# zchuning/repo

Measured on AMD Instinct MI355X. Metric: world-model+imagine updates/sec (B=50,L=50,64x64x3), higher is better.
Workload: dtype f32

## Files before the change

repo_amd/csrc/bconv.h:

```cpp
#pragma once
#include "bgemm.h"
#include "dconv.h"

namespace repo {

template <class G>
struct BGeo {
  static constexpr int KSE = G::KS + (G::KS & 1);
  static constexpr int TAPS = G::KS * KSE;
  static constexpr int KKE = (TAPS + 7) & ~7;
  static constexpr int BPG = KKE / 8;
  static constexpr bool ODD = (G::WB & 1) != 0;
  static constexpr int WBE = ODD ? ((G::WB + 3) & ~3) : G::WB;
  static constexpr int CBP = G::CB + (G::CB & 1);
};

template <int BM_, int BN_, int CK_, int WM_, int WN_>
struct BTile {
  static constexpr int BM = BM_, BN = BN_, CK = CK_, WM = WM_, WN = WN_;
  static constexpr int TM = BM / (32 * WM), TN = BN / (32 * WN);
  static constexpr int NT = WM * WN * 64;
  static_assert(TM >= 1 && TN >= 1 && BM % (32 * WM) == 0 && BN % (32 * WN) == 0 && CK % 2 == 0, "tile / wave grid mismatch");
};

template <class G, class T>
struct BPack {
  static constexpr int NBLK = (T::CK / 2) * BGeo<G>::BPG;
  static constexpr int NSL = BGeo<G>::CBP / T::CK;
  static constexpr int MT = (G::CS + T::BM - 1) / T::BM;
  static constexpr int WPLANE = NBLK * 2 * T::BM * 16;
  static constexpr int CHUNK_BYTES = 3 * WPLANE;
  static constexpr size_t BYTES = (size_t)MT * NSL * CHUNK_BYTES;
  static constexpr size_t BYTES_U8 = BYTES + (size_t)((G::CS * 4 + 255) & ~255);
  static_assert(BGeo<G>::CBP % T::CK == 0, "channel chunk must divide the (pair-padded) channel count");
};

struct BPackArgs {
  const float* w;
  char* wp;
  const float* bias;
};

template <class G, class T, bool U8 = false>
__global__ __launch_bounds__(256) void bconv_pack_kernel(BPackArgs p) {
  typedef BGeo<G> BG;
  typedef BPack<G, T> P;
  const int total = P::MT * P::NSL * P::NBLK * 2 * T::BM;
  if (U8) {
    float* fb = reinterpret_cast<float*>(p.wp + P::BYTES);
    for (int cs = blockIdx.x * 256 + threadIdx.x; cs < G::CS; cs += gridDim.x * 256) {
      double s = 0.0;
      for (int k = 0; k < G::CB * G::KK; ++k) s += (double)p.w[(size_t)cs * G::CB * G::KK + k];
      fb[cs] = (float)((double)(p.bias ? p.bias[cs] : 0.f) - s);
    }
  }
  for (int i = blockIdx.x * 256 + threadIdx.x; i < total; i += gridDim.x * 256) {
    int r = i;
    const int m = r % T::BM;
    r /= T::BM;
    const int h = r & 1;
    r >>= 1;
    const int blk = r % P::NBLK;
    r /= P::NBLK;
    const int t = r % P::NSL, mt = r / P::NSL;
    const int g = blk / BG::BPG, b = blk % BG::BPG;
    const int cs = mt * T::BM + m, cb = t * T::CK + 2 * g + h;
    float v[8];
#pragma unroll
    for (int j = 0; j < 8; ++j) {
      const int q = 8 * b + j, ky = q / BG::KSE, kx = q % BG::KSE;
      v[j] = (q < BG::TAPS && kx < G::KS && cs < G::CS && cb < G::CB) ? p.w[((size_t)cs * G::CB + cb) * G::KK + ky * G::KS + kx] : 0.f;
      if (U8) v[j] *= 2.f / 255.f;
    }
    unsigned pl[3][4];
#pragma unroll
    for (int e = 0; e < 4; ++e) bg_split3(v[2 * e], v[2 * e + 1], pl[0][e], pl[1][e], pl[2][e]);
    char* dst = p.wp + ((size_t)mt * P::NSL + t) * P::CHUNK_BYTES + ((blk * 2 + h) * T::BM + m) * 16;
#pragma unroll
    for (int q3 = 0; q3 < 3; ++q3)
      *reinterpret_cast<u32x4s*>(dst + q3 * P::WPLANE) = u32x4s{pl[q3][0], pl[q3][1], pl[q3][2], pl[q3][3]};
  }
}

template <class G, class T, class BigT = float, int NPROD = 6>
__global__ __launch_bounds__(T::NT) void bconv_down_kernel(DownArgs p) {
  typedef BGeo<G> BG;
  typedef BPack<G, T> P;
  constexpr bool U8 = std::is_same<BigT, uint8_t>::value;
  static_assert(U8 ? (NPROD == 3 || NPROD == 2) : (NPROD == 6 || NPROD == 3), "products per block");
  constexpr int NWPL = U8 ? NPROD : BgProd<U8 ? 6 : NPROD>::PLANES;
  constexpr int NPL = U8 ? 1 : NWPL;
  static_assert(BG::CBP == G::CB || P::NSL == 1, "a padded channel count: one chunk (the phantom channel is chunk-local)");
  static_assert(!U8 || !BG::ODD, "uint8 frames: even row pitch");
  constexpr bool ODD = BG::ODD;
  constexpr int WBE = BG::WBE;
  constexpr int BM = T::BM, BN = T::BN, CK = T::CK, NT = T::NT, TM = T::TM, TN = T::TN;
  constexpr int NBLK = P::NBLK, NSL = P::NSL, WPLANE = P::WPLANE;
  constexpr int ROWS_FULL = 2 * (G::HS - 1) + G::KS;
  constexpr int LENFULL = (ROWS_FULL * G::WB + 3) & ~3;
  constexpr int NIMG_MAX = (BN - 1) / G::PS + 2;
  constexpr int PLMAX = cmin(NIMG_MAX * LENFULL,
                             ((2 * (BN / G::WS + 2) + NIMG_MAX * (G::KS - 2)) * G::WB + 4 * NIMG_MAX + 3) & ~3);
  constexpr int PLV = PLMAX / 4;
  constexpr int LENFULL_E = ODD ? ROWS_FULL * WBE : LENFULL;
  constexpr int PLMAX_E = ODD ? cmin(NIMG_MAX * LENFULL_E, ((2 * (BN / G::WS + 2) + NIMG_MAX * (G::KS - 2)) * WBE + 3) & ~3)
                              : PLMAX;
  constexpr int PPLANE = (CK * PLMAX_E * 2 + 15) & ~15;
  constexpr bool QROW = ODD;
  static_assert(!ODD || WBE % 4 == 0, "padded pitch: whole quads per row");
  constexpr int PLV_E = PLMAX_E / 4;
  constexpr int W_NV = NWPL * NBLK * 2 * BM;
  constexpr int W_PER = (W_NV + NT - 1) / NT, P_PER = (CK * (QROW ? PLV_E : PLV) + NT - 1) / NT;
  constexpr int EPI_FLOATS = (NT / 64) * 32 * 36 + (NT / 64) * TM * 32;
  constexpr int LDS_BYTES = cmax(3 * WPLANE + (U8 ? 1 : 3) * PPLANE + 64, 4 * EPI_FLOATS);
  __shared__ __attribute__((aligned(16))) char lds[LDS_BYTES];
  char* Wl = lds;
  char* Pl = lds + 3 * WPLANE;

  const int tid = threadIdx.x;
  const int lane = tid & 63;
  const int wid = __builtin_amdgcn_readfirstlane(tid >> 6);
  const int wm = wid / T::WN, wn = wid % T::WN;
  const int li = lane & 31, lh = lane >> 5;

  const int Ntot = p.nimg * G::PS;
  const int n0 = xcd_tile(blockIdx.x, gridDim.x) * BN, m0 = blockIdx.y * BM;
  const int nlast = min(n0 + BN, Ntot) - 1;
  const int ia = n0 / G::PS, ib = nlast / G::PS;
  const int fa = (n0 % G::PS) / G::WS, lb = (nlast % G::PS) / G::WS;
  const int la_ = (ia == ib) ? lb : G::HS - 1;
  const int lenA = ((2 * (la_ - fa) + G::KS) * G::WB + 3) & ~3;
  auto span_start = [&](int i) __attribute__((always_inline)) { return i == ia ? 0 : lenA + (i - ia - 1) * LENFULL; };
  const int PL = span_start(ib) + (ib == ia ? lenA : ((2 * lb + G::KS) * G::WB + 3) & ~3);
  const int lenA_e = (2 * (la_ - fa) + G::KS) * WBE;
  auto span_start_e = [&](int i) __attribute__((always_inline)) {
    return ODD ? (i == ia ? 0 : lenA_e + (i - ia - 1) * LENFULL_E) : span_start(i);
  };

  const __amdgpu_buffer_rsrc_t rbig = make_rsrc(p.big, p.big_bytes), rw = make_rsrc(p.w, p.w_bytes);

  unsigned poff[P_PER];
  int plds[P_PER];
#pragma unroll
  for (int j = 0; j < P_PER; ++j) {
    if (QROW) {
      const int v = tid + j * NT, c = v / PLV_E, qe = (v % PLV_E) * 4;
      int i, rel;
      if (qe < lenA_e) {
        i = ia;
        rel = qe;
      } else {
        i = ia + 1 + (qe - lenA_e) / LENFULL_E;
        rel = (qe - lenA_e) % LENFULL_E;
      }
      const int rows_i = (i == ia) ? 2 * (la_ - fa) + G::KS : (i == ib ? 2 * lb + G::KS : ROWS_FULL);
      const int r = rel / WBE, col = rel % WBE;
      const bool act = c < CK && i <= ib && r < rows_i;
      const int f = (i == ia) ? fa : 0;
      poff[j] = act ? 4u * (unsigned)((i * G::CB + c) * G::PB + (2 * f + r) * G::WB + col) : kOobOffset;
      plds[j] = act ? 2 * (c * PLMAX_E + span_start_e(i) + rel) : -1;
      continue;
    }
    const int v = tid + j * NT, c = v / PLV, q = (v % PLV) * 4;
    const bool act = c < CK && q < PL;
    int i, rel;
    if (q < lenA) {
      i = ia;
      rel = q;
    } else {
      i = ia + 1 + (q - lenA) / LENFULL;
      rel = (q - lenA) % LENFULL;
    }
    const int f = (i == ia) ? fa : 0;
    poff[j] = (act && c < G::CB) ? (unsigned)sizeof(BigT) * (unsigned)((i * G::CB + c) * G::PB + 2 * f * G::WB + rel) : kOobOffset;
    plds[j] = act ? 2 * (c * PLMAX_E + q) : -1;
  }
  constexpr unsigned P_STEP = (unsigned)sizeof(BigT) * CK * G::PB;
  const unsigned wbase = (unsigned)(blockIdx.y * NSL) * (unsigned)P::CHUNK_BYTES;

  int bbh[TN];
#pragma unroll
  for (int j = 0; j < TN; ++j) {
    const int n = min(n0 + (wn * TN + j) * 32 + li, Ntot - 1);
    const int i = n / G::PS, pix = n % G::PS;
    const int f = (i == ia) ? fa : 0;
    bbh[j] = 2 * (span_start_e(i) + 2 * (pix / G::WS - f) * WBE + 2 * (pix % G::WS) + lh * PLMAX_E);
  }
  const int abase = (lh * BM + wm * (TM * 32) + li) * 16;

  f32x16 acc[TM][TN];
#pragma unroll
  for (int i = 0; i < TM; ++i)
#pragma unroll
    for (int j = 0; j < TN; ++j)
#pragma unroll
      for (int r = 0; r < 16; ++r) acc[i][j][r] = 0.f;

  f32x4 rwv[W_PER];
  typename Patch4<BigT>::raw_t rpv[P_PER];
  auto gload = [&](int t) __attribute__((always_inline)) {
#pragma unroll
    for (int j = 0; j < W_PER; ++j) {
      const int v = tid + j * NT;
      rwv[j] = VecLoad<4>::load(rw, ((W_NV % NT == 0) || v < W_NV) ? wbase + (unsigned)t * P::CHUNK_BYTES + 16u * v : kOobOffset);
    }
#pragma unroll
    for (int j = 0; j < P_PER; ++j)
      rpv[j] = Patch4<BigT>::load(rbig, poff[j] == kOobOffset ? kOobOffset : poff[j] + (unsigned)t * P_STEP);
  };
  auto lstore = [&]() __attribute__((always_inline)) {
#pragma unroll
    for (int j = 0; j < W_PER; ++j) {
      const int v = tid + j * NT;
      if ((W_NV % NT == 0) || v < W_NV) *reinterpret_cast<f32x4*>(Wl + 16 * v) = rwv[j];
    }
#pragma unroll
    for (int j = 0; j < P_PER; ++j)
      if (plds[j] >= 0) {
        if constexpr (U8) {
          const unsigned v = rpv[j];
          const unsigned f0 = __builtin_bit_cast(unsigned, (float)(v & 0xffu)), f1 = __builtin_bit_cast(unsigned, (float)((v >> 8) & 0xffu));
          const unsigned f2 = __builtin_bit_cast(unsigned, (float)((v >> 16) & 0xffu)), f3 = __builtin_bit_cast(unsigned, (float)(v >> 24));
          *reinterpret_cast<bg_u32x2*>(Pl + plds[j]) = bg_u32x2{(f0 >> 16) | (f1 & 0xffff0000u), (f2 >> 16) | (f3 & 0xffff0000u)};
        } else {
          unsigned a1, a2, a3, b1, b2, b3;
          bg_split3(rpv[j][0], rpv[j][1], a1, a2, a3);
          bg_split3(rpv[j][2], rpv[j][3], b1, b2, b3);
          *reinterpret_cast<bg_u32x2*>(Pl + plds[j]) = bg_u32x2{a1, b1};
          *reinterpret_cast<bg_u32x2*>(Pl + PPLANE + plds[j]) = bg_u32x2{a2, b2};
          if constexpr (NPL > 2) *reinterpret_cast<bg_u32x2*>(Pl + 2 * PPLANE + plds[j]) = bg_u32x2{a3, b3};
        }
      }
  };
  auto qoff = [](int g, int q) constexpr {
    const int ky = q / BG::KSE, kx = q % BG::KSE;
    return (q < BG::TAPS && kx < G::KS) ? 2 * (2 * g * PLMAX_E + ky * WBE + kx) : 2 * (2 * g * PLMAX_E);
  };
  auto compute = [&]() __attribute__((always_inline)) {
#pragma unroll
    for (int blk = 0; blk < NBLK; ++blk) {
      const int g = blk / BG::BPG, b = blk % BG::BPG;
      bg_bf16x8 fa[TM][3], fb[TN][NPL];
#pragma unroll
      for (int pl = 0; pl < NWPL; ++pl) {
#pragma unroll
        for (int i = 0; i < TM; ++i)
          fa[i][pl] = *reinterpret_cast<const bg_bf16x8*>(Wl + pl * WPLANE + blk * (2 * BM * 16) + abase + i * 32 * 16);
#pragma unroll
        for (int j = 0; j < (pl < NPL ? TN : 0); ++j) {
          const char* pb = Pl + pl * PPLANE + bbh[j];
          u32x4s d;
#pragma unroll
          for (int pp = 0; pp < 4; ++pp) d[pp] = *reinterpret_cast<const unsigned*>(pb + qoff(g, 8 * b + 2 * pp));
          fb[j][pl] = __builtin_bit_cast(bg_bf16x8, d);
        }
      }
#pragma unroll
      for (int i = 0; i < TM; ++i)
#pragma unroll
        for (int j = 0; j < TN; ++j) {
          f32x16 c = acc[i][j];
          if constexpr (U8) {
            if constexpr (NPROD == 3) c = __builtin_amdgcn_mfma_f32_32x32x16_bf16(fa[i][2], fb[j][0], c, 0, 0, 0);
            c = __builtin_amdgcn_mfma_f32_32x32x16_bf16(fa[i][1], fb[j][0], c, 0, 0, 0);
            c = __builtin_amdgcn_mfma_f32_32x32x16_bf16(fa[i][0], fb[j][0], c, 0, 0, 0);
          } else if constexpr (NPROD == 3) {
            c = __builtin_amdgcn_mfma_f32_32x32x16_bf16(fa[i][0], fb[j][1], c, 0, 0, 0);
            c = __builtin_amdgcn_mfma_f32_32x32x16_bf16(fa[i][1], fb[j][0], c, 0, 0, 0);
            c = __builtin_amdgcn_mfma_f32_32x32x16_bf16(fa[i][0], fb[j][0], c, 0, 0, 0);
          } else {
            c = __builtin_amdgcn_mfma_f32_32x32x16_bf16(fa[i][1], fb[j][NPL > 1 ? 1 : 0], c, 0, 0, 0);
            c = __builtin_amdgcn_mfma_f32_32x32x16_bf16(fa[i][0], fb[j][NPL > 2 ? 2 : 0], c, 0, 0, 0);
            c = __builtin_amdgcn_mfma_f32_32x32x16_bf16(fa[i][2], fb[j][0], c, 0, 0, 0);
            c = __builtin_amdgcn_mfma_f32_32x32x16_bf16(fa[i][0], fb[j][NPL > 1 ? 1 : 0], c, 0, 0, 0);
            c = __builtin_amdgcn_mfma_f32_32x32x16_bf16(fa[i][1], fb[j][0], c, 0, 0, 0);
            c = __builtin_amdgcn_mfma_f32_32x32x16_bf16(fa[i][0], fb[j][0], c, 0, 0, 0);
          }
          acc[i][j] = c;
        }
    }
  };

  gload(0);
  if (ODD) {
    for (int i = tid; i < NPL * PPLANE / 16; i += NT) reinterpret_cast<f32x4*>(Pl)[i] = f32x4{0.f, 0.f, 0.f, 0.f};
    __syncthreads();
  }
  lstore();
  __syncthreads();
  for (int t = 0; t < NSL; ++t) {
    if (t + 1 < NSL) gload(t + 1);
#ifndef BC_NO_COMPUTE
    compute();
#endif
    __syncthreads();
    if (t + 1 < NSL) {
#ifndef BC_NO_STAGE
      lstore();
#endif
      __syncthreads();
    }
  }
  dconv_down_epilogue<G, T>(p, reinterpret_cast<float*>(lds), acc, n0, m0, Ntot);
}

template <class G, class T, class BigT = float, int NPROD = 6>
inline int launch_bconv_down(const DownArgs& a, const float* w, char* pack, hipStream_t s) {
  typedef BPack<G, T> P;
  constexpr bool U8 = std::is_same<BigT, uint8_t>::value;
  const int total = P::MT * P::NSL * P::NBLK * 2 * T::BM;
  hipLaunchKernelGGL((bconv_pack_kernel<G, T, U8>), dim3((unsigned)((total + 255) / 256)), dim3(256), 0, s, BPackArgs{w, pack, a.bias});
  hipError_t e = hipGetLastError();
  if (e != hipSuccess) return (int)e;
  DownArgs b = a;
  b.w = reinterpret_cast<const float*>(pack);
  b.w_bytes = (unsigned)P::BYTES;
  if (U8) b.bias = reinterpret_cast<const float*>(pack + P::BYTES);
  const long gx = ((long)a.nimg * G::PS + T::BN - 1) / T::BN, gy = P::MT;
  hipLaunchKernelGGL((bconv_down_kernel<G, T, BigT, NPROD>), dim3((unsigned)gx, (unsigned)gy), dim3(T::NT), 0, s, b);
  e = hipGetLastError();
  return e == hipSuccess ? REPO_OK : (int)e;
}

}
```

repo_amd/csrc/conv.hip:

```cpp
#include <stdlib.h>
#include <string.h>

#include <algorithm>
#include <type_traits>

#include "igemm.h"
#include "dconv.h"
#include "uconv.h"
#include "dconv_up.h"
#include "bconv.h"
#include "buconv.h"
#include "bwgrad.h"
#include "bdec4.h"
#include "twgrad.h"
#include "tconv_up.h"
#include "tconv_down.h"

namespace repo {

static thread_local int t_bconv_enabled = 1;

static thread_local int t_conv_precision = -1;
static int env_conv_precision() {
  static const int mode = [] {
// ... 258 lines not shown
      float* p = dw + (size_t)m * Ncols + n;
      *p = accumulate ? *p + s : s;
    } else if (db) {
      db[m] = accumulate ? db[m] + s : s;
    }
  }
}

__global__ void partial_sum_rows_kernel(const float* __restrict__ parts, int n, float* __restrict__ out, float scale,
                                        int accumulate) {
  __shared__ float red[16];
  const float* row = parts + (size_t)blockIdx.x * n;
  float s = 0.f;
  for (int i = threadIdx.x; i < n; i += blockDim.x) s += row[i];
  s = block_sum(s, red);
  if (threadIdx.x == 0) out[blockIdx.x] = accumulate ? out[blockIdx.x] + scale * s : scale * s;
}

__global__ void partial_sum_kernel(const float* __restrict__ parts, int n, float* __restrict__ out, int accumulate) {
  __shared__ float red[16];
  float s = 0.f;
  for (int i = threadIdx.x; i < n; i += blockDim.x) s += parts[i];
  s = block_sum(s, red);
  if (threadIdx.x == 0) *out = accumulate ? *out + s : s;
}

__global__ void channel_sum_kernel(const float* __restrict__ x, int nimg, int C, int P, int imgs_per_split,
                                   float* __restrict__ parts) {
  __shared__ float red[16];
  const int c = blockIdx.x, s = blockIdx.y;
  const int i0 = s * imgs_per_split, i1 = min(nimg, i0 + imgs_per_split);
  const int nt = blockDim.x;
  const int dq = nt / P, dr = nt % P;
  int img = i0 + (int)threadIdx.x / P, p = (int)threadIdx.x % P;
  float a0 = 0.f, a1 = 0.f;
  const size_t cstride = (size_t)C * P;
  const float* base = x + (size_t)c * P;
  while (img < i1) {
    a0 += base[img * cstride + p];
    p += dr;
    img += dq;
    if (p >= P) {
      p -= P;
      ++img;
    }
    if (img >= i1) break;
    a1 += base[img * cstride + p];
    p += dr;
    img += dq;
    if (p >= P) {
      p -= P;
      ++img;
    }
  }
  const float acc = block_sum(a0 + a1, red);
  if (threadIdx.x == 0) parts[s * C + c] = acc;
}
__global__ void channel_sum_final_kernel(const float* __restrict__ parts, int splits, int C, float* __restrict__ out,
                                         int accumulate) {
  const int lane = threadIdx.x & 63;
  const int c = blockIdx.x * (blockDim.x >> 6) + (threadIdx.x >> 6);
  if (c >= C) return;
  float s = 0.f;
  for (int z = lane; z < splits; z += 64) s += parts[z * C + c];
  s = wave_sum(s);
  if (lane == 0) out[c] = accumulate ? out[c] + s : s;
}

__global__ void relu_mask_kernel(int64_t n, const float* __restrict__ dy, const float* __restrict__ h,
                                 float* __restrict__ y) {
  const int64_t stride = (int64_t)gridDim.x * blockDim.x;
  for (int64_t i = (int64_t)blockIdx.x * blockDim.x + threadIdx.x; i < n; i += stride) y[i] = h[i] > 0.f ? dy[i] : 0.f;
}

struct Off {};
template <class T> constexpr bool kOn = !std::is_same<T, Off>::value;

template <class Down_, class Wgrad_, int WGT_>
struct LayerFp32 {
  using Down = Down_; using Wgrad = Wgrad_; static constexpr int WGT = WGT_;
  using DownLat = Off;
  using DownBf = Off;
  using DownBfU8 = Off;
  using DownTcd = Off;
  static bool down_tcd_takes(int, bool, bool) { return false; }
  using UpScatter = Off;
  using UpBfScatter = Off;
  using DirectUp = Off;
  static constexpr bool UpTconv = false;
  using WgradBf = Off;
  static constexpr int TwNBK = 0, TwNPW = 4;
  static constexpr bool TwDbig = true;
};

template <class G> struct Layer;
template <> struct Layer<GEnc1> : LayerFp32<DTile<32, 512, 3, 1, 8>, WTile<32, 64, 1, 2, 1, 4, 2>, 3072> {
  using DownBfU8 = BTile<32, 512, 4, 1, 8>;
};
template <> struct Layer<GEnc2> : LayerFp32<DTile<64, 128, 2, 2, 2>, WTile<64, 128, 2, 2, 1, 7, 2>, 768> {
  using DownLat = DTile<32, 128, 4, 1, 4>;
  using DownBf = BTile<64, 256, 4, 1, 4>;
  using DownTcd = TcdGeoE2;
  static bool down_tcd_takes(int epi, bool, bool) { return epi == REPO_EPI_RELU; }
  using UpScatter = SConf<GEnc2, 1, 8>;
  using UpBfScatter = BSConf<GEnc2, 1, 4>;
  static constexpr bool UpTconv = true;
  static constexpr int TwNBK = 2, TwNPW = 8;
};
template <> struct Layer<GEnc3> : LayerFp32<DTile<128, 128, 2, 2, 2>, WTile<64, 128, 2, 2, 2, 6>, 1024> {
  using DownLat = DTile<32, 128, 8, 1, 4>;
  using DownBf = BTile<128, 128, 4, 2, 2>;
  using UpScatter = SConf<GEnc3, 4, 2>;
  using UpBfScatter = BSConf<GEnc3, 4, 4>;
  using WgradBf = WTile<64, 256, 1, 4, 1, 6>;
};
template <> struct Layer<GEnc4> : LayerFp32<DTile<32, 64, 2, 1, 2>, WTile<64, 128, 2, 2, 8, 2>, 768> {
  using DownLat = DTile<32, 128, 8, 1, 4>;
  using DownBf = BTile<128, 64, 4, 2, 2>;
  using UpScatter = SConf<GEnc4, 8, 1>;
  using UpBfScatter = BSConf<GEnc4, 8, 2>;
};
template <> struct Layer<GDec2> : LayerFp32<DTile<128, 128, 4, 2, 4, 1>, WTile<64, 128, 2, 2, 4, 5>, 1536> {
  using DownBf = BTile<64, 128, 2, 1, 4>;
  using UpScatter = SConf<GDec2, 5, 2>;
  using UpBfScatter = BSConf<GDec2, 5, 4>;
};
template <> struct Layer<GDec3> : LayerFp32<DTile<64, 128, 2, 2, 2>, WTile<64, 128, 2, 2, 1, 7>, 2048> {
  using DownBf = BTile<64, 256, 2, 1, 4>;
  using DownTcd = TcdGeo;
  static bool down_tcd_takes(int epi, bool has_bias, bool wants_cmask) {
    return (epi == REPO_EPI_NONE || epi == REPO_EPI_MUL_DRELU) && !has_bias && !wants_cmask;
  }
  using UpScatter = SConf<GDec3, 1, 6>;
  using UpBfScatter = BSConf<GDec3, 1, 4>;
  using WgradBf = WTile<64, 128, 1, 4, 1, 7>;
  static constexpr int TwNBK = 2;
};
template <> struct Layer<GDec4> : LayerFp32<DTile<32, 256, 3, 1, 8>, WTile<32, 128, 1, 4, 1, 2>, 1536> {};
template <> struct Layer<GX1> : LayerFp32<DTile<32, 512, 3, 1, 8>, WTile<32, 64, 1, 2, 1, 2, 2>, 3072> {};
template <> struct Layer<GX2> : LayerFp32<DTile<64, 128, 2, 2, 2>, WTile<64, 128, 2, 2, 1, 3, 2>, 1536> {
  using DirectUp = DTile<128, 128, 8, 2, 4>;
};
template <> struct Layer<GX3> : LayerFp32<DTile<128, 128, 2, 2, 2>, WTile<64, 128, 2, 2, 1, 7>, 1024> {
  using UpScatter = SConf<GX3, 1, 2>;
};
template <> struct Layer<GX4> : LayerFp32<DTile<64, 128, 2, 2, 2>, WTile<64, 128, 2, 2, 2, 6>, 1024> {
  using UpScatter = SConf<GX4, 4, 1>;
};
template <> struct Layer<GY4> : LayerFp32<DTile<32, 256, 2, 1, 4>, WTile<32, 128, 1, 4, 1, 2>, 1536> {
  using DirectUp = DTile<64, 256, 4, 2, 4>;
};
template <> struct Layer<GY5> : LayerFp32<DTile<32, 512, 3, 1, 8>, WTile<32, 64, 1, 2, 1, 2>, 1536> {};
template <> struct Layer<GT4> : LayerFp32<DTile<32, 256, 3, 1, 8>, WTile<32, 128, 1, 4, 1, 2>, 1536> {
  using DirectUp = DTile<32, 256, 4, 1, 8>;
};

template <class G> struct Route : Layer<G> {
#if defined(TCD_DISABLE)
  using DownTcd = Off;
#elif defined(TCD_NO_ENC2)
  using DownTcd = std::conditional_t<std::is_same<G, GEnc2>::value, Off, typename Layer<G>::DownTcd>;
#endif
#ifdef TCU_DISABLE
  static constexpr bool UpTconv = false;
#endif
#ifdef TW_DISABLE
  static constexpr int TwNBK = 0;
#endif
#ifdef TW_NO_DBIG
  static constexpr bool TwDbig = false;
#endif
};
template <class G> using DownLatTile = std::conditional_t<kOn<typename Route<G>::DownLat>, typename Route<G>::DownLat, typename Route<G>::Down>;
template <class G, class BigT> using DownBfTile = std::conditional_t<std::is_same<BigT, float>::value, typename Route<G>::DownBf, typename Route<G>::DownBfU8>;

constexpr size_t round256(size_t b) { return (b + 255) & ~(size_t)255; }

enum class DownEngine { Fp32Lat, Fp32, Bf16, Tcd };
struct DownPlan {
  DownEngine engine;
  long tiles;
  size_t pack_bytes;
  size_t parts_bytes;
  bool high;
  size_t need() const { return pack_bytes + parts_bytes; }
};
template <class G, class BigT>
static DownPlan down_plan(int64_t nimg, int epi, bool has_bias, bool wants_dbias, bool wants_cmask, size_t ws_have) {
  using R = Route<G>;
  using BT = DownBfTile<G, BigT>;
  const long px = nimg * (long)G::PS;
  auto plan = [&](DownEngine e, long bn, size_t pack) {
    const long tiles = (px + bn - 1) / bn;
    return DownPlan{e, tiles, pack, wants_dbias ? (size_t)tiles * G::CS * sizeof(float) : 0, conv_precision_high()};
  };
  if constexpr (kOn<BT>) {
    if (t_bconv_enabled && px > 512) {
      using P = BPack<G, BT>;
      constexpr size_t pack = round256(std::is_same<BigT, float>::value ? P::BYTES : P::BYTES_U8);
      DownPlan b = plan(DownEngine::Bf16, BT::BN, pack);
      if constexpr (kOn<typename R::DownTcd>) {
        static_assert(std::is_same<BigT, float>::value && R::DownTcd::PACK_BYTES <= pack,
                      "tconv_down: float frames; its pack fits the room of the bf16x6 kernel's");
        if (nimg >= 32 && !wants_dbias && R::down_tcd_takes(epi, has_bias, wants_cmask)) b.engine = DownEngine::Tcd;
      }
      if (ws_have >= b.need()) return b;
    }
  }
  return px <= 512 ? plan(DownEngine::Fp32Lat, DownLatTile<G>::BN, 0) : plan(DownEngine::Fp32, R::Down::BN, 0);
}
template <class G>
static size_t conv_down_ws_bytes(int64_t nimg) {
  const DownPlan f = down_plan<G, float>(nimg, REPO_EPI_NONE, false, true, false, SIZE_MAX);
  const DownPlan u = down_plan<G, uint8_t>(nimg, REPO_EPI_NONE, false, true, false, SIZE_MAX);
  return std::max(f.pack_bytes, u.pack_bytes) + std::max(f.parts_bytes, u.parts_bytes);
}

template <class G, class BigT>
static int conv_down_t(int64_t nimg, const BigT* big, const float* w, const float* bias, float* small, int epi,
                       const float* aux, float* dbias, int accumulate_dbias, unsigned char* cmask, void* ws,
                       size_t ws_bytes, hipStream_t s) {
  if (cmask && G::CS % 4 != 0) return REPO_E_BADARG;
  if (nimg * (int64_t)G::CB * G::PB >= kMaxBufElems || nimg * (int64_t)G::CS * G::PS >= kMaxBufElems) return REPO_E_SHAPE;
  const size_t ws_have = ws ? ws_bytes : 0;
  const DownPlan p = down_plan<G, BigT>(nimg, epi, bias != nullptr, dbias != nullptr, cmask != nullptr, ws_have);
  if (ws_have < p.need()) return REPO_E_WS_TOO_SMALL;
  float* parts = dbias ? (float*)((char*)ws + p.pack_bytes) : nullptr;
  DownArgs a{big, w, bias, aux, small, (int)nimg, epi, (unsigned)(nimg * G::CB * G::PB * sizeof(BigT)),
             (unsigned)(G::CS * G::CB * G::KK * sizeof(float)), parts, cmask};
  int rc = REPO_E_BADARG;
  switch (p.engine) {
    case DownEngine::Tcd:
      if constexpr (kOn<typename Route<G>::DownTcd>)
        rc = p.high ? launch_tconv_down<typename Route<G>::DownTcd, 3>(a, w, (char*)ws, s)
                    : launch_tconv_down<typename Route<G>::DownTcd, 6>(a, w, (char*)ws, s);
      break;
    case DownEngine::Bf16:
      if constexpr (kOn<DownBfTile<G, BigT>>) {
        constexpr int NFULL = std::is_same<BigT, float>::value ? 6 : 3;
        rc = p.high ? launch_bconv_down<G, DownBfTile<G, BigT>, BigT, NFULL == 6 ? 3 : 2>(a, w, (char*)ws, s)
                    : launch_bconv_down<G, DownBfTile<G, BigT>, BigT, NFULL>(a, w, (char*)ws, s);
      }
      break;
    case DownEngine::Fp32Lat: rc = launch_dconv_down<G, BigT, DownLatTile<G>>(a, s); break;
    case DownEngine::Fp32: rc = launch_dconv_down<G, BigT, typename Route<G>::Down>(a, s); break;
  }
  if (rc || !dbias) return rc;
  hipLaunchKernelGGL(channel_sum_final_kernel, dim3(cdiv(G::CS, 4)), dim3(256), 0, s, (const float*)parts, (int)p.tiles,
                     (int)G::CS, dbias, accumulate_dbias);
  REPO_CHECK_LAUNCH();
  return REPO_OK;
}

enum class UpEngine { Tconv, BfScatter, Direct, Scatter, Merged };
struct UpPlan {
  UpEngine engine;
  UpEngine base;
  bool tcu_live;
  size_t tcu_off;
  size_t need;
  size_t total;
  bool high;
};
template <class G>
static UpPlan up_plan(int64_t nimg, int epi, size_t ws_have) {
  using R = Route<G>;
  using UC = typename R::UpScatter;
  using BC = typename R::UpBfScatter;
  static_assert(!kOn<BC> || kOn<UC>, "the bf16x6 scatter kernel has an fp32 twin (repo_debug_bconv(0))");
  static_assert(!kOn<typename R::DirectUp> || !kOn<UC>, "the direct kernel or the scatter kernels");
  static_assert(!R::UpTconv || kOn<BC>, "the gather-form kernel follows the debug switch of the bf16x6 kernels");
  UpPlan p{UpEngine::Merged, UpEngine::Merged, false, 0, 0, 0, conv_precision_high()};
  size_t room = 0;
  if constexpr (kOn<BC>) {
    p.base = t_bconv_enabled ? UpEngine::BfScatter : UpEngine::Scatter;
    p.need = t_bconv_enabled ? BC::PACK_BYTES : UC::PACK_FLOATS * sizeof(float);
    room = std::max(BC::PACK_BYTES, UC::PACK_FLOATS * sizeof(float));
  } else if constexpr (kOn<typename R::DirectUp>) {
    p.base = UpEngine::Direct, p.need = room = UpGeo<G>::PACK_FLOATS * sizeof(float);
  } else if constexpr (kOn<UC>) {
    p.base = UpEngine::Scatter, p.need = room = UC::PACK_FLOATS * sizeof(float);
  }
  p.engine = p.base;
  p.tcu_off = round256(room);
  p.total = R::UpTconv ? p.tcu_off + kTcuPackBytes : room;
  p.tcu_live = R::UpTconv && t_bconv_enabled;
  const bool epi_ok = epi == REPO_EPI_NONE || epi == REPO_EPI_MUL_DRELU || epi == REPO_EPI_MUL_CMASK;
  if (p.tcu_live && epi_ok && nimg >= 4 && ws_have >= p.total) {
    p.engine = UpEngine::Tconv;
    p.need = p.total;
  }
  return p;
}

template <class G>
static int conv_up_pack_t(const float* w, void* ws, size_t ws_bytes, hipStream_t s) {
  using R = Route<G>;
  const size_t ws_have = ws ? ws_bytes : 0;
  const UpPlan p = up_plan<G>(0, REPO_EPI_NONE, ws_have);
  if (ws_have < (p.tcu_live ? p.total : p.need)) return REPO_E_WS_TOO_SMALL;
  if (p.tcu_live)
    if (const int rc = launch_tconv_up_pack(w, (char*)ws + p.tcu_off, s)) return rc;
  if constexpr (kOn<typename R::UpBfScatter>)
    if (p.base == UpEngine::BfScatter) return launch_buconv_pack<G, typename R::UpBfScatter>(w, ws, ws_bytes, s);
  if constexpr (kOn<typename R::DirectUp>) return launch_dconv_up_pack<G>(w, ws, ws_bytes, s);
  else if constexpr (kOn<typename R::UpScatter>) return launch_uconv_pack<G, typename R::UpScatter>(w, ws, ws_bytes, s);
  else return REPO_OK;
}

template <class G>
static int conv_up_t(int64_t nimg, const float* small, const float* w, const float* bias, float* big, int epi,
                     const float* aux, int packed, void* ws, size_t ws_bytes, hipStream_t s) {
  if (nimg * (int64_t)G::CB * G::PB >= kMaxBufElems || nimg * (int64_t)G::CS * G::PS >= kMaxBufElems) return REPO_E_SHAPE;
  using R = Route<G>;
  if (epi == REPO_EPI_MUL_CMASK && (!kOn<typename R::UpScatter> || G::CB % 4 != 0)) return REPO_E_BADARG;
  if (epi == REPO_EPI_FILM_RELU && !kOn<typename R::UpScatter>) return REPO_E_BADARG;
  const size_t ws_have = ws ? ws_bytes : 0;
  const UpPlan p = up_plan<G>(nimg, epi, ws_have);
  if (ws_have < p.need) return REPO_E_WS_TOO_SMALL;
  if constexpr (R::UpTconv)
    if (p.engine == UpEngine::Tconv) {
      char* pack = (char*)ws + p.tcu_off;
// ... 369 lines not shown
```

repo_amd/csrc/dconv.h:

```cpp
#pragma once
#include "vgemm.h"

namespace repo {

template <int BM_, int BN_, int CK_, int WM_, int WN_, int LDWPAD_ = 2>
struct DTile {
  static constexpr int BM = BM_, BN = BN_, CK = CK_, WM = WM_, WN = WN_, LDWPAD = LDWPAD_;
  static constexpr int TM = BM / (32 * WM), TN = BN / (32 * WN);
  static constexpr int NT = WM * WN * 64;
  static_assert(TM >= 1 && TN >= 1 && BM % (32 * WM) == 0 && BN % (32 * WN) == 0, "tile / wave grid mismatch");
};

#ifdef REPO_IGEMM_STAMPS
#define REPO_STAMP_FLUSH(nslices)                                              \
  do {                                                                         \
    REPO_STAMP(4);                                                             \
    if ((threadIdx.x & 63) == 0 && blockIdx.x % 16 == 0) {                     \
      for (int i_ = 0; i_ < 6; ++i_) atomicAdd(&g_igemm_stamps[i_], st_[i_]);  \
      atomicAdd(&g_igemm_stamps[6], 1ull);                                     \
      atomicAdd(&g_igemm_stamps[7], (unsigned long long)(nslices));            \
    }                                                                          \
  } while (0)
#else
#define REPO_STAMP_FLUSH(nslices)
// ... 100 lines not shown
            float fsc = 1.f, fsh = 0.f;
            if (p.epi == REPO_EPI_FILM_RELU) {
              fsc = p.aux[(size_t)(2 * img) * G::CS + m];
              fsh = p.aux[(size_t)(2 * img + 1) * G::CS + m];
            }
#pragma unroll
            for (int e = 0; e < 4; ++e) {
              float x = v[e] + bv;
              if (p.epi == REPO_EPI_RELU) x = fmaxf(x, 0.f);
              else if (p.epi == REPO_EPI_MUL_DRELU || p.epi == REPO_EPI_MUL_MASK4) x = a4[e] > 0.f ? x : 0.f;
              else if (p.epi == REPO_EPI_FILM_RELU) x = fmaxf(fmaf(fsc, x, fsh), 0.f);
              v[e] = x;
            }
            qs = (v[0] + v[1]) + (v[2] + v[3]);
            __builtin_amdgcn_raw_buffer_store_b128(__builtin_bit_cast(u32x4s, v), rout, 4u * o, 0, 0);
          } else {
#pragma unroll
            for (int e = 0; e < 4; ++e) {
              const int ne = n + e;
              if (ne < Ntot) {
                const int oe = ((ne / G::PS) * G::CS + m) * G::PS + ne % G::PS;
                float x = v[e] + bv;
                if (p.epi == REPO_EPI_RELU) x = fmaxf(x, 0.f);
                else if (p.epi == REPO_EPI_FILM_RELU)
                  x = fmaxf(fmaf(p.aux[(size_t)(2 * (ne / G::PS)) * G::CS + m], x, p.aux[(size_t)(2 * (ne / G::PS) + 1) * G::CS + m]), 0.f);
                else if (p.epi == REPO_EPI_MUL_DRELU) x = p.aux[oe] > 0.f ? x : 0.f;
                else if (p.epi == REPO_EPI_MUL_MASK4)
                  x = (reinterpret_cast<const unsigned char*>(p.aux)[oe >> 2] >> (oe & 3)) & 1 ? x : 0.f;
                p.out[oe] = x;
                qs += x;
              }
            }
          }
        }
        if (p.chan_part) {
          qs += __shfl_xor(qs, 1, 64);
          qs += __shfl_xor(qs, 2, 64);
          qs += __shfl_xor(qs, 4, 64);
          csum[i][pass] += qs;
        }
      }
      if (p.cmask) {
        const int cq = lane >> 3, q = lane & 7;
        const int m4 = mt + 4 * cq, n = nb + 4 * q;
        if (m4 < G::CS && n < Ntot) {
          f32x4 rws[4];
          float bq[4];
#pragma unroll
          for (int c = 0; c < 4; ++c) {
            rws[c] = *reinterpret_cast<const f32x4*>(strip + (4 * cq + c) * EP + 4 * q);
            bq[c] = p.bias ? p.bias[m4 + c] : 0.f;
          }
#pragma unroll
          for (int e = 0; e < 4; ++e) {
            const int ne = n + e;
            if (ne < Ntot) {
              unsigned bits = 0;
#pragma unroll
              for (int c = 0; c < 4; ++c) bits |= (rws[c][e] + bq[c] > 0.f ? 1u : 0u) << c;
              p.cmask[((size_t)(ne / G::PS) * (G::CS / 4) + (m4 >> 2)) * G::PS + ne % G::PS] = (unsigned char)bits;
            }
          }
        }
      }
      __builtin_amdgcn_wave_barrier();
    }
  if (p.chan_part) {
    float* red = lds + (NT / 64) * 32 * EP;
    if ((lane & 7) == 0) {
#pragma unroll
      for (int i = 0; i < TM; ++i)
#pragma unroll
        for (int pass = 0; pass < 4; ++pass) red[wid * (TM * 32) + i * 32 + pass * 8 + (lane >> 3)] = csum[i][pass];
    }
    __syncthreads();
    if (tid < BM && m0 + tid < G::CS) {
      const int wmc = tid / (TM * 32), c = tid % (TM * 32);
      float t = 0.f;
#pragma unroll
      for (int x = 0; x < T::WN; ++x) t += red[(wmc * T::WN + x) * (TM * 32) + c];
      p.chan_part[(size_t)blockIdx.x * G::CS + m0 + tid] = t;
    }
  }
}

template <class G, class BigT, class T>
__global__ __launch_bounds__(T::NT) void dconv_down_kernel(DownArgs p) {
  constexpr int BM = T::BM, BN = T::BN, CK = T::CK, NT = T::NT, TM = T::TM, TN = T::TN;
  constexpr int KSL = CK * G::KK;
  constexpr int NSL = G::CB / CK;
  static_assert(G::CB % CK == 0 && KSL % 4 == 0, "channel chunk must divide CB and give k % 4 == 0");
  constexpr int LDW = BM + T::LDWPAD;
  constexpr int ROWS_FULL = 2 * (G::HS - 1) + G::KS;
  constexpr int LENFULL = (ROWS_FULL * G::WB + 3) & ~3;
  constexpr int NIMG_MAX = (BN - 1) / G::PS + 2;
  constexpr int PLMAX = cmin(NIMG_MAX * LENFULL,
                             ((2 * (BN / G::WS + 2) + NIMG_MAX * (G::KS - 2)) * G::WB + 4 * NIMG_MAX + 3) & ~3);
  constexpr int PLV = PLMAX / 4;
  constexpr int W_NV = BM * KSL / 4, W_KV = KSL / 4;
  constexpr int W_PER = (W_NV + NT - 1) / NT, P_PER = (CK * PLV + NT - 1) / NT;
  constexpr int NBUF = NSL > 1 ? 2 : 1;
  constexpr int EP = 36;
  __shared__ __attribute__((aligned(16))) float lds[cmax(NBUF * KSL * LDW + NBUF * CK * PLMAX, (NT / 64) * 32 * EP + (NT / 64) * TM * 32)];
  float* Wl = lds;
  float* Pl = lds + NBUF * KSL * LDW;

  const int tid = threadIdx.x;
  const int lane = tid & 63;
  const int wid = __builtin_amdgcn_readfirstlane(tid >> 6);
  const int wm = wid / T::WN, wn = wid % T::WN;
  const int li = lane & 31, lh = lane >> 5;

  const int Ntot = p.nimg * G::PS;
  const int n0 = xcd_tile(blockIdx.x, gridDim.x) * BN, m0 = blockIdx.y * BM;
  const int nlast = min(n0 + BN, Ntot) - 1;
  const int ia = n0 / G::PS, ib = nlast / G::PS;
  const int fa = (n0 % G::PS) / G::WS, lb = (nlast % G::PS) / G::WS;
  const int la_ = (ia == ib) ? lb : G::HS - 1;
  const int lenA = ((2 * (la_ - fa) + G::KS) * G::WB + 3) & ~3;
  auto span_start = [&](int i) __attribute__((always_inline)) { return i == ia ? 0 : lenA + (i - ia - 1) * LENFULL; };
  const int PL = span_start(ib) + (ib == ia ? lenA : ((2 * lb + G::KS) * G::WB + 3) & ~3);

  const __amdgpu_buffer_rsrc_t rbig = make_rsrc(p.big, p.big_bytes), rw = make_rsrc(p.w, p.w_bytes);

  unsigned woff[W_PER];
  int wlds[W_PER];
#pragma unroll
  for (int j = 0; j < W_PER; ++j) {
    const int v = tid + j * NT, kv = v % W_KV, m = v / W_KV;
    const bool act = (W_NV % NT == 0) || v < W_NV;
    woff[j] = act ? 4u * (unsigned)(min(m0 + m, G::CS - 1) * (G::CB * G::KK) + kv * 4) : kOobOffset;
    wlds[j] = act ? (kv * 4) * LDW + m : -1;
  }
  unsigned poff[P_PER];
  int plds[P_PER];
#pragma unroll
  for (int j = 0; j < P_PER; ++j) {
    const int v = tid + j * NT, c = v / PLV, q = (v % PLV) * 4;
    const bool act = c < CK && q < PL;
    int i, rel;
    if (q < lenA) {
      i = ia;
      rel = q;
    } else {
      i = ia + 1 + (q - lenA) / LENFULL;
      rel = (q - lenA) % LENFULL;
    }
    const int f = (i == ia) ? fa : 0;
    poff[j] = act ? (unsigned)Patch4<BigT>::BYTES * (unsigned)((i * G::CB + c) * G::PB + 2 * f * G::WB + rel)
                  : kOobOffset;
    plds[j] = act ? c * PLMAX + q : -1;
  }
  constexpr unsigned W_STEP = 4u * KSL, P_STEP = (unsigned)Patch4<BigT>::BYTES * CK * G::PB;

  int bbase[TN];
#pragma unroll
  for (int j = 0; j < TN; ++j) {
    const int n = min(n0 + (wn * TN + j) * 32 + li, Ntot - 1);
    const int i = n / G::PS, pix = n % G::PS;
    const int f = (i == ia) ? fa : 0;
    bbase[j] = span_start(i) + 2 * (pix / G::WS - f) * G::WB + 2 * (pix % G::WS);
  }
  int bbase1[TN];
#pragma unroll
  for (int j = 0; j < TN; ++j) bbase1[j] = bbase[j] + lh;
  const int abase = lh * LDW + wm * (TM * 32) + li;
// ... 517 lines not shown
```

Baseline: 179.3.

## Add producer/consumer staging waves with double-buffered LDS to bconv down kernel

Adds a warp-specialized variant of the bf16-split down-conv kernel. Extra staging waves do the global loads and LDS stores into a double buffer while the compute waves only run MFMA on the other buffer, with named LDS barriers between them. The variant is enabled by default for the GEnc4 layer (float frames), using a smaller channel chunk and launch bounds that request 4 waves per EU. It costs twice the staging LDS, more threads per block, and idle stager waves that must still join the epilogue barriers.

Measured after the change: 179.1. Within noise of the previous version (-0.1%).

```diff
diff --git a/repo_amd/csrc/bconv.h b/repo_amd/csrc/bconv.h
--- a/repo_amd/csrc/bconv.h
+++ b/repo_amd/csrc/bconv.h
@@ -1,6 +1,7 @@
 #pragma once
 #include "bgemm.h"
 #include "dconv.h"
+#include "rowtile.h"
 
 namespace repo {
 
@@ -15,11 +16,11 @@
   static constexpr int CBP = G::CB + (G::CB & 1);
 };
 
-template <int BM_, int BN_, int CK_, int WM_, int WN_>
+template <int BM_, int BN_, int CK_, int WM_, int WN_, int SW_ = 0, int WPE_ = 1>
 struct BTile {
-  static constexpr int BM = BM_, BN = BN_, CK = CK_, WM = WM_, WN = WN_;
+  static constexpr int BM = BM_, BN = BN_, CK = CK_, WM = WM_, WN = WN_, SW = SW_, WPE = WPE_;
   static constexpr int TM = BM / (32 * WM), TN = BN / (32 * WN);
-  static constexpr int NT = WM * WN * 64;
+  static constexpr int NT = WM * WN * 64, NTL = NT + 64 * SW;
   static_assert(TM >= 1 && TN >= 1 && BM % (32 * WM) == 0 && BN % (32 * WN) == 0 && CK % 2 == 0, "tile / wave grid mismatch");
 };
 
@@ -83,10 +84,12 @@
 }
 
 template <class G, class T, class BigT = float, int NPROD = 6>
-__global__ __launch_bounds__(T::NT) void bconv_down_kernel(DownArgs p) {
+__global__ __launch_bounds__(T::NTL, T::WPE) void bconv_down_kernel(DownArgs p) {
   typedef BGeo<G> BG;
   typedef BPack<G, T> P;
   constexpr bool U8 = std::is_same<BigT, uint8_t>::value;
+  constexpr bool STG = T::SW > 0;
+  static_assert(!STG || (!U8 && P::NSL > 1), "staging waves: float frames, more than one chunk");
   static_assert(U8 ? (NPROD == 3 || NPROD == 2) : (NPROD == 6 || NPROD == 3), "products per block");
   constexpr int NWPL = U8 ? NPROD : BgProd<U8 ? 6 : NPROD>::PLANES;
   constexpr int NPL = U8 ? 1 : NWPL;
@@ -110,16 +113,19 @@
   static_assert(!ODD || WBE % 4 == 0, "padded pitch: whole quads per row");
   constexpr int PLV_E = PLMAX_E / 4;
   constexpr int W_NV = NWPL * NBLK * 2 * BM;
-  constexpr int W_PER = (W_NV + NT - 1) / NT, P_PER = (CK * (QROW ? PLV_E : PLV) + NT - 1) / NT;
+  constexpr int NS = STG ? 64 * T::SW : NT;
+  constexpr int W_PER = (W_NV + NS - 1) / NS, P_PER = (CK * (QROW ? PLV_E : PLV) + NS - 1) / NS;
   constexpr int EPI_FLOATS = (NT / 64) * 32 * 36 + (NT / 64) * TM * 32;
-  constexpr int LDS_BYTES = cmax(3 * WPLANE + (U8 ? 1 : 3) * PPLANE + 64, 4 * EPI_FLOATS);
+  constexpr int BUF_BYTES = 3 * WPLANE + (U8 ? 1 : 3) * PPLANE + 64;
+  constexpr int LDS_BYTES = cmax((STG ? 2 : 1) * BUF_BYTES, 4 * EPI_FLOATS);
   __shared__ __attribute__((aligned(16))) char lds[LDS_BYTES];
-  char* Wl = lds;
-  char* Pl = lds + 3 * WPLANE;
+  constexpr int POFF = 3 * WPLANE;
 
   const int tid = threadIdx.x;
   const int lane = tid & 63;
   const int wid = __builtin_amdgcn_readfirstlane(tid >> 6);
+  const bool stager = !STG || wid >= NT / 64;
+  const int st = STG ? tid - NT : tid;
   const int wm = wid / T::WN, wn = wid % T::WN;
   const int li = lane & 31, lh = lane >> 5;
 
@@ -143,8 +149,13 @@
   int plds[P_PER];
 #pragma unroll
   for (int j = 0; j < P_PER; ++j) {
+    if (!stager) {
+      poff[j] = kOobOffset;
+      plds[j] = -1;
+      continue;
+    }
     if (QROW) {
-      const int v = tid + j * NT, c = v / PLV_E, qe = (v % PLV_E) * 4;
+      const int v = st + j * NS, c = v / PLV_E, qe = (v % PLV_E) * 4;
       int i, rel;
       if (qe < lenA_e) {
         i = ia;
@@ -161,7 +172,7 @@
       plds[j] = act ? 2 * (c * PLMAX_E + span_start_e(i) + rel) : -1;
       continue;
     }
-    const int v = tid + j * NT, c = v / PLV, q = (v % PLV) * 4;
+    const int v = st + j * NS, c = v / PLV, q = (v % PLV) * 4;
     const bool act = c < CK && q < PL;
     int i, rel;
     if (q < lenA) {
@@ -201,18 +212,20 @@
   auto gload = [&](int t) __attribute__((always_inline)) {
 #pragma unroll
     for (int j = 0; j < W_PER; ++j) {
-      const int v = tid + j * NT;
-      rwv[j] = VecLoad<4>::load(rw, ((W_NV % NT == 0) || v < W_NV) ? wbase + (unsigned)t * P::CHUNK_BYTES + 16u * v : kOobOffset);
+      const int v = st + j * NS;
+      rwv[j] = VecLoad<4>::load(rw, ((W_NV % NS == 0) || v < W_NV) ? wbase + (unsigned)t * P::CHUNK_BYTES + 16u * v : kOobOffset);
     }
 #pragma unroll
     for (int j = 0; j < P_PER; ++j)
       rpv[j] = Patch4<BigT>::load(rbig, poff[j] == kOobOffset ? kOobOffset : poff[j] + (unsigned)t * P_STEP);
   };
-  auto lstore = [&]() __attribute__((always_inline)) {
+  auto lstore = [&](char* buf) __attribute__((always_inline)) {
+    char* const Wl = buf;
+    char* const Pl = buf + POFF;
 #pragma unroll
     for (int j = 0; j < W_PER; ++j) {
-      const int v = tid + j * NT;
-      if ((W_NV % NT == 0) || v < W_NV) *reinterpret_cast<f32x4*>(Wl + 16 * v) = rwv[j];
+      const int v = st + j * NS;
+      if ((W_NV % NS == 0) || v < W_NV) *reinterpret_cast<f32x4*>(Wl + 16 * v) = rwv[j];
     }
 #pragma unroll
     for (int j = 0; j < P_PER; ++j)
@@ -236,7 +249,9 @@
     const int ky = q / BG::KSE, kx = q % BG::KSE;
     return (q < BG::TAPS && kx < G::KS) ? 2 * (2 * g * PLMAX_E + ky * WBE + kx) : 2 * (2 * g * PLMAX_E);
   };
-  auto compute = [&]() __attribute__((always_inline)) {
+  auto compute = [&](const char* buf) __attribute__((always_inline)) {
+    const char* const Wl = buf;
+    const char* const Pl = buf + POFF;
 #pragma unroll
     for (int blk = 0; blk < NBLK; ++blk) {
       const int g = blk / BG::BPG, b = blk % BG::BPG;
@@ -281,24 +296,68 @@
     }
   };
 
-  gload(0);
-  if (ODD) {
-    for (int i = tid; i < NPL * PPLANE / 16; i += NT) reinterpret_cast<f32x4*>(Pl)[i] = f32x4{0.f, 0.f, 0.f, 0.f};
+  if constexpr (!STG) {
+    gload(0);
+    if (ODD) {
+      for (int i = tid; i < NPL * PPLANE / 16; i += NT) reinterpret_cast<f32x4*>(lds + POFF)[i] = f32x4{0.f, 0.f, 0.f, 0.f};
+      __syncthreads();
+    }
+    lstore(lds);
     __syncthreads();
-  }
-  lstore();
-  __syncthreads();
-  for (int t = 0; t < NSL; ++t) {
-    if (t + 1 < NSL) gload(t + 1);
+    for (int t = 0; t < NSL; ++t) {
+      if (t + 1 < NSL) gload(t + 1);
 #ifndef BC_NO_COMPUTE
-    compute();
-#endif
-    __syncthreads();
-    if (t + 1 < NSL) {
+      compute(lds);
+#endif
+      __syncthreads();
+      if (t + 1 < NSL) {
 #ifndef BC_NO_STAGE
-      lstore();
-#endif
+        lstore(lds);
+#endif
+        __syncthreads();
+      }
+    }
+  } else {
+    if (stager) gload(0);
+    if (ODD) {
+      for (int i = tid; i < 2 * (NPL * PPLANE / 16); i += T::NTL) {
+        const int b = i / (NPL * PPLANE / 16), r = i % (NPL * PPLANE / 16);
+        reinterpret_cast<f32x4*>(lds + b * BUF_BYTES + POFF)[r] = f32x4{0.f, 0.f, 0.f, 0.f};
+      }
       __syncthreads();
+    }
+    if (stager) {
+      lstore(lds);
+      gload(1);
+      lds_barrier();
+      auto step = [&](int t, char* other) __attribute__((always_inline)) {
+        if (t + 1 < NSL) {
+#ifndef BC_NO_STAGE
+          lstore(other);
+          if (t + 2 < NSL) gload(t + 2);
+#endif
+        }
+        lds_barrier();
+      };
+      for (int t = 0; t < NSL; t += 2) {
+        step(t, lds + BUF_BYTES);
+        if (t + 1 < NSL) step(t + 1, lds);
+      }
+      dconv_down_epilogue_idle(p);
+      return;
+    }
+    lds_barrier();
+    for (int t = 0; t < NSL; t += 2) {
+#ifndef BC_NO_COMPUTE
+      compute(lds);
+#endif
+      lds_barrier();
+      if (t + 1 < NSL) {
+#ifndef BC_NO_COMPUTE
+        compute(lds + BUF_BYTES);
+#endif
+        lds_barrier();
+      }
     }
   }
   dconv_down_epilogue<G, T>(p, reinterpret_cast<float*>(lds), acc, n0, m0, Ntot);
@@ -317,7 +376,7 @@
   b.w_bytes = (unsigned)P::BYTES;
   if (U8) b.bias = reinterpret_cast<const float*>(pack + P::BYTES);
   const long gx = ((long)a.nimg * G::PS + T::BN - 1) / T::BN, gy = P::MT;
-  hipLaunchKernelGGL((bconv_down_kernel<G, T, BigT, NPROD>), dim3((unsigned)gx, (unsigned)gy), dim3(T::NT), 0, s, b);
+  hipLaunchKernelGGL((bconv_down_kernel<G, T, BigT, NPROD>), dim3((unsigned)gx, (unsigned)gy), dim3(T::NTL), 0, s, b);
   e = hipGetLastError();
   return e == hipSuccess ? REPO_OK : (int)e;
 }
diff --git a/repo_amd/csrc/conv.hip b/repo_amd/csrc/conv.hip
--- a/repo_amd/csrc/conv.hip
+++ b/repo_amd/csrc/conv.hip
@@ -364,6 +364,7 @@
   using DownLat = Off;
   using DownBf = Off;
   using DownBfU8 = Off;
+  using DownBfStaged = Off;
   using DownTcd = Off;
   static bool down_tcd_takes(int, bool, bool) { return false; }
   using UpScatter = Off;
@@ -399,6 +400,7 @@
 template <> struct Layer<GEnc4> : LayerFp32<DTile<32, 64, 2, 1, 2>, WTile<64, 128, 2, 2, 8, 2>, 768> {
   using DownLat = DTile<32, 128, 8, 1, 4>;
   using DownBf = BTile<128, 64, 4, 2, 2>;
+  using DownBfStaged = BTile<128, 64, 2, 2, 2, 4, 4>;
   using UpScatter = SConf<GEnc4, 8, 1>;
   using UpBfScatter = BSConf<GEnc4, 8, 2>;
 };
@@ -455,6 +457,11 @@
 };
 template <class G> using DownLatTile = std::conditional_t<kOn<typename Route<G>::DownLat>, typename Route<G>::DownLat, typename Route<G>::Down>;
 template <class G, class BigT> using DownBfTile = std::conditional_t<std::is_same<BigT, float>::value, typename Route<G>::DownBf, typename Route<G>::DownBfU8>;
+
+static bool bconv_staging_enabled() {
+  const char* e = getenv("REPO_BCONV_STAGING");
+  return !(e && e[0] == '0' && e[1] == 0);
+}
 
 constexpr size_t round256(size_t b) { return (b + 255) & ~(size_t)255; }
 
@@ -520,6 +527,16 @@
     case DownEngine::Bf16:
       if constexpr (kOn<DownBfTile<G, BigT>>) {
         constexpr int NFULL = std::is_same<BigT, float>::value ? 6 : 3;
+        if constexpr (std::is_same<BigT, float>::value && kOn<typename Route<G>::DownBfStaged>) {
+          using BT = DownBfTile<G, BigT>;
+          using ST = typename Route<G>::DownBfStaged;
+          static_assert(ST::BM == BT::BM && ST::BN == BT::BN && BPack<G, ST>::BYTES == BPack<G, BT>::BYTES && BPack<G, ST>::MT == BPack<G, BT>::MT,
+                        "the staging-wave form keeps the plan's tiles, grid and pack size");
+          if (bconv_staging_enabled()) {
+            rc = p.high ? launch_bconv_down<G, ST, BigT, 3>(a, w, (char*)ws, s) : launch_bconv_down<G, ST, BigT, 6>(a, w, (char*)ws, s);
+            break;
+          }
+        }
         rc = p.high ? launch_bconv_down<G, DownBfTile<G, BigT>, BigT, NFULL == 6 ? 3 : 2>(a, w, (char*)ws, s)
                     : launch_bconv_down<G, DownBfTile<G, BigT>, BigT, NFULL>(a, w, (char*)ws, s);
       }
diff --git a/repo_amd/csrc/dconv.h b/repo_amd/csrc/dconv.h
--- a/repo_amd/csrc/dconv.h
+++ b/repo_amd/csrc/dconv.h
@@ -206,6 +206,11 @@
       p.chan_part[(size_t)blockIdx.x * G::CS + m0 + tid] = t;
     }
   }
+}
+
+__device__ __forceinline__ void dconv_down_epilogue_idle(const DownArgs& p) {
+  __syncthreads();
+  if (p.chan_part) __syncthreads();
 }
 
 template <class G, class BigT, class T>
```
